# CliMA/ClimateParameterizations.jl

Measured on AMD Instinct MI355X. Metric: column-timesteps/sec (fwd+adjoint), 32-level wind-mixing NDE, higher is better.
Workload: dtype f32

## Files before the change

climateparameterizations.jl_amd/csrc/engine_regtile.hip:

```cpp
#include <cstdlib>
#include "engine_regtile.h"
#include "kernel_select.h"
#include "split_bf16.h"

typedef float f32x16 __attribute__((ext_vector_type(16)));

#ifdef COLNDE_STAMPS
__device__ unsigned long long g_rt_stamps[16];
#define RT_STAMP_DECL unsigned long long rs_t0 = 0, rs_acc[8] = {0, 0, 0, 0, 0, 0, 0, 0}; const unsigned long long rs_kk = __builtin_amdgcn_s_memtime(), rs_rr = __builtin_amdgcn_s_memrealtime()
#define RT_STAMP_BEGIN() do { __builtin_amdgcn_sched_barrier(0); rs_t0 = __builtin_amdgcn_s_memtime(); __builtin_amdgcn_sched_barrier(0); } while (0)
#define RT_STAMP(i) do { __builtin_amdgcn_sched_barrier(0); unsigned long long t_ = __builtin_amdgcn_s_memtime(); rs_acc[i] += t_ - rs_t0; rs_t0 = t_; __builtin_amdgcn_sched_barrier(0); } while (0)
#define RT_STAMP_FLUSH() do { if (blockIdx.x == 0 && threadIdx.x == 0) { for (int q_ = 0; q_ < 8; q_++) g_rt_stamps[q_] = rs_acc[q_]; g_rt_stamps[8] = __builtin_amdgcn_s_memtime() - rs_kk; g_rt_stamps[9] = __builtin_amdgcn_s_memrealtime() - rs_rr; } } while (0)
#else
#define RT_STAMP_DECL
#define RT_STAMP_BEGIN()
#define RT_STAMP(i)
#define RT_STAMP_FLUSH()
#endif
typedef float f32x4v __attribute__((ext_vector_type(4)));
typedef float f32x2v __attribute__((ext_vector_type(2)));

#define RHO0(r) (((r) & 3) + 8 * ((r) >> 2))
#ifndef RT16_WAVES
#define RT16_WAVES 8
// ... 803 lines not shown
                gg[r] = (r == 0 && h == 0) ? 0.0f : (d[r] - dd[r]) * 32.0f;
                sums[q] += d[r] * d[r];
                sums[3 + q] += gg[r] * gg[r];
            }
            if (add) {
                const f32x16 gu_ = shift_up(gg, h, 0.0f);
#pragma unroll
                for (int r = 0; r < 16; r++)
                    lam[RT_LAM(q * 16 + r, lane)] += 2.0f * lw.w[q] * d[r] + 2.0f * lw.w[3 + q] * 32.0f * (gg[r] - gu_[r]);
            }
        }
    };
    inject(0, false);

    auto load_z1 = [&](int step, int st, int n, f32x16 (&Z)[2], f32x16 (&Dz)[2]) {
        size_t rec = (size_t)step * 4 + st;
#ifdef RT_ABL_Z1_CACHED
        { int z_ = 0; asm volatile("" : "+v"(z_)); rec = (size_t)z_; }
#endif
        const float* srcz = tpz + rec * RT_TAPEZ;
        auto fill = [&](const float* src, f32x16 (&T)[2]) {
#pragma unroll
            for (int t = (13 * n) >> 2; t <= (13 * n + 12) >> 2; t++)
#pragma unroll
                for (int c = 0; c < 2; c++) {
                    const f32x4v v = RT_TAPE_LOAD4(src + (2 * t + c) * 256);
#pragma unroll
                    for (int e = 0; e < 4; e++) {
                        const int G = 2 * (4 * t + e - 13 * n) + c;
                        if ((4 * t + e) / 13 == n && G < 25) T[G >> 4][G & 15] = v[e];
                    }
                }
        };
        fill(srcz, Z);
        if (RT_ZRICH) fill(srcz + RT_TAPEZ_HALF, Dz);
    };

    auto load_z2 = [&](int step, int st, int n, f32x16& Z) {
        const float* srcz = tpz + ((size_t)step * 4 + st) * RT_TAPEZ + RT_Z2OFF + n * 3 * 256;
#pragma unroll
        for (int grp = 0; grp < 3; grp++) {
            const f32x4v v = RT_TAPE_LOAD4(srcz + grp * 256);
#pragma unroll
            for (int e = 0; e < 4; e++) Z[4 * grp + e] = (4 * grp + e < 10) ? v[e] : 0.0f;
        }
#pragma unroll
        for (int r = 12; r < 16; r++) Z[r] = 0.0f;
    };

    auto load_x = [&](int step, int st) {
        const float* src = tp + ((size_t)step * 4 + st) * 3072;
#pragma unroll
        for (int q = 0; q < 3; q++)
#pragma unroll
            for (int g = 0; g < 4; g++) {
                const f32x4v v = RT_TAPE_LOAD4(src + (q * 4 + g) * 256);
                X[q][4 * g] = v[0]; X[q][4 * g + 1] = v[1]; X[q][4 * g + 2] = v[2]; X[q][4 * g + 3] = v[3];
            }
    };

    for (int iv = n_save - 2; iv >= 0; iv--) {
        const float dt = (save_times[iv + 1] - save_times[iv]) / (float)substeps;
        inject(iv + 1, true);
        for (int s = substeps - 1; s >= 0; s--) {
            const int step = iv * substeps + s;
#pragma nounroll
            for (int st = 3; st >= 0; st--) {
                const float cwl = (st == 0 || st == 3) ? dt / 6.0f : dt / 3.0f;
                const float cwx = st == 3 ? 0.0f : (st == 2 ? dt : 0.5f * dt);
                RT_STAMP_BEGIN();
                f32x16 A1[2], D1[2];
                f32x16 A1n[2], D1n[2];
#pragma unroll
                for (int r = 9; r < 16; r++) { A1[1][r] = 0.0f; D1[1][r] = 0.0f; A1n[1][r] = 0.0f; D1n[1][r] = 0.0f; }
                load_x(step, st);
                f32x16 dOk[3];
                {
                    f32x16 kb[3];
#pragma unroll
                    for (int q = 0; q < 3; q++)
#pragma unroll
                        for (int r = 0; r < 16; r++) kb[q][r] = cwl * lam[RT_LAM(q * 16 + r, lane)] + cwx * xb[q][r];
                    rt_physics_vjp(m, X, kb, h, xb);
#pragma unroll
                    for (int q = 0; q < 3; q++) dOk[q] = kb[q];
                }
                RT_STAMP(0);
                float* dst = tp2 + ((size_t)step * 4 + st) * RT_TAPE2;
                float carry[2] = {0.0f, 0.0f};
#pragma unroll
                for (int n = 0; n < 3; n++) {
                    const f32x16 dOn = dOk[n];
                    if (ZT) {
                        if (n == 0) {
                            load_z1(step, st, 0, A1, D1);
#ifdef COLNDE_STAMPS
                            asm volatile("s_waitcnt vmcnt(0)" ::: "memory");
                            RT_STAMP(7);
#endif
                            if (!RT_ZRICH) {
#pragma unroll
                                for (int G = 0; G < 24; G += 4) rt_act_pair4_at<ACT>(A1, D1, G);
                                rt_act_pair_at<ACT>(A1, D1, 24);
                            }
                        }
                    } else {
#pragma unroll
                        for (int t = 0; t < 2; t++) {
                            f32x16 acc;
#pragma unroll
                            for (int r = 0; r < 16; r++) acc[r] = (t * 16 + r < 25) ? wl[RT_B1C + n * 50 + 2 * (t * 16 + r) + h] : 0.0f;
                            const int base = a1n[t] + n * 50 * RT_LD1;
                            acc = rt_chain<48, RT_ADJ_CH>(wl, acc, [=](int k) { return base + (k >> 4) * 32 + RHO0(k & 15); },
                                                          [&](int k) { return X[k >> 4][k & 15]; });
#pragma unroll
                            for (int r = 0; r < 16; r++) {
                                float av = 0.0f, dv = 0.0f;
                                if (t * 16 + r < 25) rt_act_pair<ACT>(acc[r], av, dv);
                                A1[t][r] = av;
                                D1[t][r] = dv;
                            }
                        }
                    }
                    RT_STAMP(1);
                    f32x16 Z2;
                    if (ZT && RT_Z2TAPE) load_z2(step, st, n, Z2);
                    else {
                        f32x16 acc;
#pragma unroll
                        for (int r = 0; r < 16; r++) acc[r] = r < 10 ? wl[RT_B2C + n * 20 + 2 * r + h] : 0.0f;
                        const int base2 = a2b + n * 20 * RT_LD2;
                        Z2 = rt_chain<25, 5>(wl, acc, [=](int k) { return base2 + 2 * k; },
                                             [&](int k) { return A1[k >> 4][k & 15]; });
                    }
                    RT_STAMP(2);
                    {
#ifndef RT_ABL_NO_OUTER
                        const f32x16 TA = rt_transpose(tb, dOn, wbase, rbase);
                        b3acc[n] += rt_sum16(TA);
#endif
                        f32x16 A2;
#pragma unroll
                        for (int r = 0; r < 16; r += 4) {
                            f32x2v a0 = {0.0f, 0.0f}, d0 = {0.0f, 0.0f}, a1 = {0.0f, 0.0f}, d1 = {0.0f, 0.0f};
                            if (r < 8) rt_act_pair4<ACT>((f32x2v){Z2[r], Z2[r + 1]}, (f32x2v){Z2[r + 2], Z2[r + 3]}, a0, d0, a1, d1);
                            else if (r == 8) rt_act_pair2<ACT>((f32x2v){Z2[8], Z2[9]}, a0, d0);
                            A2[r] = a0.x; A2[r + 1] = a0.y; A2[r + 2] = a1.x; A2[r + 3] = a1.y;
                            Z2[r] = d0.x; Z2[r + 1] = d0.y; Z2[r + 2] = d1.x; Z2[r + 3] = d1.y;
                        }
#ifndef RT_ABL_NO_OUTER
                        const f32x16 TB = rt_transpose(tb, A2, wbase, rbase);
#ifdef RT_OUTER_SPLIT
                        if constexpr (SPLIT) gW3[n] = rt_outer_split(gW3[n], rt_split_tile(TA), rt_split_tile(TB));
                        else
#endif
                        gW3[n] = rt_outer(gW3[n], TA, TB);
#else
                        gW3[n][0] += A2[0];
#endif
                    }
                    {
                        const int base = b3T + n * 31 * RT_LD3;
                        const f32x16 da = rt_chain<16, 8>(wl, (f32x16)(0.0f), [=](int k) { return base + RHO0(k) * RT_LD3; },
                                                          [&](int k) { return dOn[k]; });
#pragma unroll
                        for (int r = 0; r < 16; r++) Z2[r] = da[r] * Z2[r];
                    }
                    RT_STAMP(3);
                    if (ZT && n < 2) load_z1(step, st, n + 1, A1n, D1n);
#ifndef RT_LPIPE
#define RT_LPIPE 1
#endif
                    u32x4 Lr[9];
                    const u32x4* lg = nullptr;
                    if constexpr (SPLIT) {
                        int lz = lane;
                        asm volatile("" : "+v"(lz));
                        lg = reinterpret_cast<const u32x4*>(wimg + RT_ASIMG_OFF + RT_ASIMG_L) + n * 9 * 64 + lz;
#pragma unroll
                        for (int u = 0; u < (RT_LPIPE ? 3 : 9); u++) Lr[u] = lg[u * 64];
                    }
#ifdef RT_ABL_NO_OUTER
                    gW2[n][0][0] += Z2[0] * A1[0][0]; gW2[n][1][0] += Z2[1] * A1[1][0];
#else
                    {
                        const f32x16 TA = rt_transpose(tb, Z2, wbase, rbase);
                        b2acc[n] += rt_sum16(TA);
#ifdef RT_OUTER_SPLIT
                        Bf3x2 TAs;
                        if constexpr (SPLIT) TAs = rt_split_tile(TA);
#endif
#pragma unroll
                        for (int t = 0; t < 2; t++) {
                            const f32x16 TB = rt_transpose(tb, A1[t], wbase, rbase);
#ifdef RT_OUTER_SPLIT
                            if constexpr (SPLIT) gW2[n][t] = rt_outer_split(gW2[n][t], TAs, rt_split_tile(TB));
                            else
#endif
                            gW2[n][t] = rt_outer(gW2[n][t], TA, TB);
                        }
                    }
#endif
                    RT_STAMP(4);
#pragma unroll
                    for (int t = 0; t < 2; t++) {
                        const int base = b2T[t] + n * 20 * RT_LD2;
                        const f32x16 da = rt_chain<10, 10>(wl, (f32x16)(0.0f), [=](int k) { return base + 2 * k * RT_LD2; },
                                                           [&](int k) { return Z2[k]; });
#pragma unroll
                        for (int r = 0; r < 16; r++) D1[t][r] = da[r] * D1[t][r];
                    }
                    auto store_delta = [&] {
#pragma unroll
                    for (int g = 0; g < 25; g++) {
                        const int G = 25 * n + g;
                        if ((G & 3) == 0 && g + 3 < 25) {
                            const f32x4v v = {D1[g >> 4][g & 15], D1[(g + 1) >> 4][(g + 1) & 15], D1[(g + 2) >> 4][(g + 2) & 15],
                                              D1[(g + 3) >> 4][(g + 3) & 15]};
                            RT_NT_STORE4(dst + (G >> 2) * 256, v);
                        }
                    }
                    if (n == 0) carry[0] = D1[1][8];
                    if (n == 1) {
                        RT_NT_STORE4(dst + 6 * 256, ((f32x4v){carry[0], D1[0][0], D1[0][1], D1[0][2]}));
                        carry[0] = D1[1][7];
                        carry[1] = D1[1][8];
                    }
                    if (n == 2) {
                        RT_NT_STORE4(dst + 12 * 256, ((f32x4v){carry[0], carry[1], D1[0][0], D1[0][1]}));
                        RT_NT_STORE4(dst + 18 * 256, ((f32x4v){D1[1][6], D1[1][7], D1[1][8], 0.0f}));
                    }
                    };
#ifndef RT_ABL_NO_TAPE2
                    if constexpr (!SPLIT) store_delta();
#endif
                    RT_STAMP(5);
                    if constexpr (SPLIT) {
                        const u32x4* hm = reinterpret_cast<const u32x4*>(rt_smem) + lane;
#pragma unroll
                        for (int c = 0; c < 3; c++) {
                            if (RT_LPIPE && c < 2) {
#pragma unroll
                                for (int u = 0; u < 3; u++) Lr[3 * (c + 1) + u] = lg[(3 * (c + 1) + u) * 64];
                            }
                            float d8[8];
#pragma unroll
                            for (int u = 0; u < 8; u++) d8[u] = D1[(8 * c + u) >> 4][(8 * c + u) & 15];
                            const Bf3 Bc = bf3_split8(d8);
#pragma unroll
                            for (int q = 0; q < 3; q++) {
                                const int G = n * 9 + c * 3 + q, slot = c * 3 + q;
                                const u32x4 Ah = hm[(G * 2) * 64], Am = hm[(G * 2 + 1) * 64];
                                if (ZT && !RT_ZRICH && n < 2 && slot >= 2) {
                                    if (slot < 8) rt_act_pair4_at<ACT>(A1n, D1n, 4 * (slot - 2));
                                    else rt_act_pair_at<ACT>(A1n, D1n, 24);
                                }
                                xb[q] = mfma_bf(Am, Bc.m, xb[q]);
                                xb[q] = mfma_bf(Ah, Bc.l, xb[q]);
                                xb[q] = mfma_bf(Am, Bc.h, xb[q]);
                                xb[q] = mfma_bf(Ah, Bc.m, xb[q]);
                                xb[q] = mfma_bf(Ah, Bc.h, xb[q]);
                                xb[q] = mfma_bf(Lr[slot], Bc.h, xb[q]);
                                RT_SCHED_FENCE();
                            }
                        }
                        const float* left = rt_smem + RT_ASIMG_LEFT + (n * 2 + h) * 96 + i_;
#pragma unroll
                        for (int q = 0; q < 3; q++) xb[q] = mfma32(left[q * 32], D1[1][8], xb[q]);
                        store_delta();
                    } else
#pragma unroll
                    for (int q = 0; q < 3; q++) {
                        const int base = b1T + q * 32 + n * 50 * RT_LD1;
                        xb[q] = rt_chain_fill<25, 5>(wl, xb[q], [=](int g) { return base + 2 * g * RT_LD1; },
                                                     [&](int g) { return D1[g >> 4][g & 15]; },
                                                     [&](int c) {
                                                         if (ZT && !RT_ZRICH && n < 2 && (q > 0 || c > 0)) {
#pragma unroll
                                                             for (int G = 0; G < 24; G += 4)
                                                                 if ((G >> 2) * 2 + 2 == q * 5 + c)
                                                                     rt_act_pair4_at<ACT>(A1n, D1n, G);
                                                             if (q * 5 + c == 14) rt_act_pair_at<ACT>(A1n, D1n, 24);
                                                         }
                                                     });
                    }
                    if (ZT && n < 2) {
#pragma unroll
                        for (int t = 0; t < 2; t++) { A1[t] = A1n[t]; D1[t] = D1n[t]; }
                    }
                }
                RT_STAMP(6);
#pragma unroll
                for (int q = 0; q < 3; q++) xbs[q] += xb[q];
            }
#pragma unroll
            for (int q = 0; q < 3; q++) {
#pragma unroll
                for (int r = 0; r < 16; r++) lam[RT_LAM(q * 16 + r, lane)] += xbs[q][r];
                xbs[q] = (f32x16)(0.0f);
            }
        }
    }

#ifndef COLNDE_STAMPS_FWD
    RT_STAMP_FLUSH();
#endif
    float* out = slab + (size_t)tile * (m.n_params + 8);
    const int r_j = (j & 3) + 4 * (j >> 3), h_j = (j >> 2) & 1;
#pragma unroll
    for (int n = 0; n < 3; n++) {
        if (r_j < 10) {
            const int f2 = 2 * r_j + h_j;
#pragma unroll
            for (int r = 0; r < 16; r++) {
                const int face = RHO0(r) + 4 * h;
                if (face >= 1) out[n * m.net_size + m.w_off[2] + f2 * 31 + face - 1] = gW3[n][r];
            }
        }
#pragma unroll
        for (int t = 0; t < 2; t++) {
            const int Gp = t * 16 + r_j;
            if (Gp < 25) {
                const int f1 = 2 * Gp + h_j;
#pragma unroll
                for (int r = 0; r < 10; r++) out[n * m.net_size + m.w_off[1] + f1 * 20 + 2 * r + h] = gW2[n][t][r];
            }
        }
        const float s2 = b2acc[n] + swap32(b2acc[n], h), s3 = b3acc[n] + swap32(b3acc[n], h);
        if (h == 0) {
            if (r_i < 10) out[n * m.net_size + m.b_off[1] + 2 * r_i + h_i] = s2;
            if (i_ >= 1) out[n * m.net_size + m.b_off[2] + i_ - 1] = s3;
        }
    }
#pragma unroll
    for (int q = 0; q < 6; q++) {
        float v = sums[q];
        for (int off = 32; off > 0; off >>= 1) v += __shfl_down(v, off);
        if (lane == 0) out[m.n_params + q] = v;
    }
}

#define RT_DW1_LDS (4 * 2048)
__global__ void __launch_bounds__(256)
rt_dw1_kernel(DevModel m, const float* __restrict__ tape, const float* __restrict__ tape2, long n_items,
              float* __restrict__ slab_rows) {
    const int lane = threadIdx.x & 63, wave = __builtin_amdgcn_readfirstlane(threadIdx.x >> 6);
    const int j = lane & 31, h = lane >> 5;
    float* buf = rt_smem + wave * RT_DW1_LDS;
    const long gw = (long)blockIdx.x * RT_WAVES + wave, GW = (long)gridDim.x * RT_WAVES;
    f32x16 gW1[5][3];
#pragma unroll
    for (int mt = 0; mt < 5; mt++)
#pragma unroll
        for (int q = 0; q < 3; q++) gW1[mt][q] = (f32x16)(0.0f);
    float b1acc[5] = {0, 0, 0, 0, 0};
    const int NQ = gw < n_items ? 4 * (int)((n_items - gw + GW - 1) / GW) : 0;
    const int soff = ((lane >> 1) & 3) * 256 + ((lane & 1) * 32 + (lane >> 3)) * 4;
    auto issue = [&](int Q, int ring) {
        const int Qc = Q < NQ ? Q : NQ - 1;
        const size_t item = (size_t)(gw + (long)(Qc >> 2) * GW);
        const float* sx = tape + item * 3072 + soff + (Qc & 3) * 32;
        const float* sz = tape2 + item * RT_TAPE2 + soff + (Qc & 3) * 32;
#pragma unroll
        for (int T = 0; T < 3; T++) __builtin_amdgcn_global_load_lds(sx + T * 1024, buf + ring * 2048 + T * 256, 16, 0, RT_DMA_AUX);
#pragma unroll
        for (int T = 0; T < 5; T++) __builtin_amdgcn_global_load_lds(sz + T * 1024, buf + ring * 2048 + (3 + T) * 256, 16, 0, RT_DMA_AUX);
    };
    const float* rd = buf + h * 32 + j;
    float op[2][8][4];
    auto read_set = [&](int set, int ring) {
#pragma unroll
        for (int T = 0; T < 8; T++)
#pragma unroll
            for (int s = 0; s < 4; s++) op[set][T][s] = rd[ring * 2048 + T * 256 + 64 * s];
    };
    if (NQ > 0) {
        issue(0, 0);
        issue(1, 1);
        issue(2, 2);
        asm volatile("s_waitcnt vmcnt(16)" ::: "memory");
        read_set(0, 0);
    }
    for (int Qb = 0; Qb < NQ; Qb += 4) {
#pragma unroll
        for (int u = 0; u < 4; u++) {
            const int cur = u & 1;
#pragma unroll
            for (int s = 0; s < 4; s++)
#pragma unroll
                for (int q = 0; q < 3; q++) gW1[0][q] = mfma32(op[cur][3][s], op[cur][q][s], gW1[0][q]);
            b1acc[0] += (op[cur][3][0] + op[cur][3][1]) + (op[cur][3][2] + op[cur][3][3]);
            __builtin_amdgcn_sched_barrier(0);
            issue(Qb + u + 3, (u + 3) & 3);
            asm volatile("s_waitcnt vmcnt(16)" ::: "memory");
            read_set(cur ^ 1, (u + 1) & 3);
            __builtin_amdgcn_sched_barrier(0);
#pragma unroll
            for (int mt = 1; mt < 5; mt++) {
#pragma unroll
                for (int s = 0; s < 4; s++)
#pragma unroll
                    for (int q = 0; q < 3; q++) gW1[mt][q] = mfma32(op[cur][3 + mt][s], op[cur][q][s], gW1[mt][q]);
                b1acc[mt] += (op[cur][3 + mt][0] + op[cur][3 + mt][1]) + (op[cur][3 + mt][2] + op[cur][3 + mt][3]);
            }
            __builtin_amdgcn_sched_barrier(0);
        }
    }
    asm volatile("s_waitcnt vmcnt(0)" ::: "memory");
    float* out = slab_rows + (size_t)gw * (m.n_params + 8);
#pragma unroll
    for (int mt = 0; mt < 5; mt++) {
#pragma unroll
        for (int r = 0; r < 16; r++) {
            const int G = mt * 16 + r;
            if (G < 75) {
                const int n = G / 25, f = 2 * (G % 25) + h;
#pragma unroll
                for (int q = 0; q < 3; q++) out[n * m.net_size + m.w_off[0] + (q * 32 + j) * 50 + f] = gW1[mt][q][r];
            }
        }
        const float s1 = b1acc[mt] + swap32(b1acc[mt], h);
        const int r_j = (j & 3) + 4 * (j >> 3), h_j = (j >> 2) & 1;
        const int G = mt * 16 + r_j;
        if (h == 0 && G < 75) out[(G / 25) * m.net_size + m.b_off[0] + 2 * (G % 25) + h_j] = s1;
    }
}

__global__ void __launch_bounds__(256)
rt_dw1_split_kernel(DevModel m, const float* __restrict__ tape, const float* __restrict__ tape2, long n_items,
                    float* __restrict__ slab_rows) {
    const int lane = threadIdx.x & 63, wave = __builtin_amdgcn_readfirstlane(threadIdx.x >> 6);
    const int j = lane & 31, h = lane >> 5;
    float* buf = rt_smem + wave * RT_DW1_LDS;
    const long gw = (long)blockIdx.x * RT_WAVES + wave, GW = (long)gridDim.x * RT_WAVES;
    f32x16 gW1[5][3];
#pragma unroll
    for (int mt = 0; mt < 5; mt++)
#pragma unroll
        for (int q = 0; q < 3; q++) gW1[mt][q] = (f32x16)(0.0f);
    float b1acc[5] = {0, 0, 0, 0, 0};
    const int NQ = gw < n_items ? 4 * (int)((n_items - gw + GW - 1) / GW) : 0;
    const int soff = ((lane >> 1) & 3) * 256 + ((lane & 1) * 32 + (lane >> 3)) * 4;
    auto issue = [&](int Q, int ring) {
        const int Qc = Q < NQ ? Q : NQ - 1;
        const size_t item = (size_t)(gw + (long)(Qc >> 2) * GW);
        const float* sx = tape + item * 3072 + soff + (Qc & 3) * 32;
        const float* sz = tape2 + item * RT_TAPE2 + soff + (Qc & 3) * 32;
#pragma unroll
        for (int T = 0; T < 3; T++) __builtin_amdgcn_global_load_lds(sx + T * 1024, buf + ring * 2048 + T * 256, 16, 0, RT_DMA_AUX);
#pragma unroll
        for (int T = 0; T < 5; T++) __builtin_amdgcn_global_load_lds(sz + T * 1024, buf + ring * 2048 + (3 + T) * 256, 16, 0, RT_DMA_AUX);
    };
    const float* rd = buf + h * 2048 + j;
    float raw[2][8][8];
    auto read_half = [&](int set, int slot0) {
#pragma unroll
        for (int T = 0; T < 8; T++)
#pragma unroll
            for (int c = 0; c < 8; c++) raw[set][T][c] = rd[slot0 * 2048 + T * 256 + c * 32];
    };
    if (NQ > 0) {
        issue(0, 0);
        issue(1, 1);
        issue(2, 2);
        issue(3, 3);
        asm volatile("s_waitcnt vmcnt(16)" ::: "memory");
        read_half(0, 0);
        asm volatile("s_waitcnt lgkmcnt(0)" ::: "memory");
        issue(4, 0);
        issue(5, 1);
    }
    for (int Qb = 0; Qb < NQ; Qb += 4) {
#pragma unroll
        for (int u = 0; u < 2; u++) {
            const int cur = u;
            asm volatile("s_waitcnt vmcnt(16)" ::: "memory");
            read_half(cur ^ 1, 2 * (u ^ 1));
            __builtin_amdgcn_sched_barrier(0);
            Bf3 X[3];
#pragma unroll
            for (int q = 0; q < 3; q++) X[q] = bf3_split8(raw[cur][q]);
            __builtin_amdgcn_sched_barrier(0);
            asm volatile("s_waitcnt lgkmcnt(0)" ::: "memory");
            issue(Qb + 2 * u + 6, 2 * (u ^ 1));
            issue(Qb + 2 * u + 7, 2 * (u ^ 1) + 1);
            __builtin_amdgcn_sched_barrier(0);
#pragma unroll
            for (int mt = 0; mt < 5; mt++) {
                const Bf3 Z = bf3_split8(raw[cur][3 + mt]);
#pragma unroll
                for (int q = 0; q < 3; q++) gW1[mt][q] = mfma_bf3(Z, X[q], gW1[mt][q]);
                const float* z = raw[cur][3 + mt];
                b1acc[mt] += ((z[0] + z[1]) + (z[2] + z[3])) + ((z[4] + z[5]) + (z[6] + z[7]));
            }
            __builtin_amdgcn_sched_barrier(0);
        }
    }
    asm volatile("s_waitcnt vmcnt(0)" ::: "memory");
    float* out = slab_rows + (size_t)gw * (m.n_params + 8);
#pragma unroll
    for (int mt = 0; mt < 5; mt++) {
#pragma unroll
        for (int r = 0; r < 16; r++) {
            const int G = mt * 16 + r;
            if (G < 75) {
                const int n = G / 25, f = 2 * (G % 25) + h;
#pragma unroll
                for (int q = 0; q < 3; q++) out[n * m.net_size + m.w_off[0] + (q * 32 + j) * 50 + f] = gW1[mt][q][r];
            }
        }
        const float s1 = b1acc[mt] + swap32(b1acc[mt], h);
        const int r_j = (j & 3) + 4 * (j >> 3), h_j = (j >> 2) & 1;
        const int G = mt * 16 + r_j;
        if (h == 0 && G < 75) out[(G / 25) * m.net_size + m.b_off[0] + 2 * (G % 25) + h_j] = s1;
    }
}

typedef float f32x4t __attribute__((ext_vector_type(4)));

__device__ __forceinline__ f32x4t mfma16t(float a, float b, f32x4t c) {
    return __builtin_amdgcn_mfma_f32_16x16x4f32(a, b, c, 0, 0, 0);
}

__device__ __forceinline__ f32x4t mfma16_bf(u32x4 a, u32x4 b, f32x4t c) {
    return __builtin_amdgcn_mfma_f32_16x16x32_bf16(__builtin_bit_cast(bf16x8, a), __builtin_bit_cast(bf16x8, b), c, 0, 0, 0);
}
__device__ __forceinline__ f32x4t mfma16_bf3(const Bf3& a, const Bf3& b, f32x4t c) {
    c = mfma16_bf(a.m, b.m, c);
    c = mfma16_bf(a.l, b.h, c);
    c = mfma16_bf(a.h, b.l, c);
    c = mfma16_bf(a.m, b.h, c);
    c = mfma16_bf(a.h, b.m, c);
    c = mfma16_bf(a.h, b.h, c);
    return c;
}
__device__ __forceinline__ Bf3 rt16_ldA(const u32x4* simg, int G, int lane) {
    Bf3 a;
    a.h = simg[(G * 3 + 0) * 64 + lane];
    a.m = simg[(G * 3 + 1) * 64 + lane];
    a.l = simg[(G * 3 + 2) * 64 + lane];
    return a;
}

__device__ __forceinline__ float rot_dn16(float x, int lane) { return __shfl(x, (lane + 48) & 63); }
__device__ __forceinline__ float rot_up16(float x, int lane) { return __shfl(x, (lane + 16) & 63); }

struct V16 { f32x4t t[2]; };

__device__ __forceinline__ V16 shift_down16(const V16& T, int lane, float below) {
    const int g = lane >> 4;
    const float r0 = rot_dn16(T.t[0][3], lane), r1 = rot_dn16(T.t[1][3], lane);
    V16 o;
    o.t[0][0] = g == 0 ? below : r0;
    o.t[1][0] = g == 0 ? r0 : r1;
#pragma unroll
    for (int tau = 0; tau < 2; tau++) { o.t[tau][1] = T.t[tau][0]; o.t[tau][2] = T.t[tau][1]; o.t[tau][3] = T.t[tau][2]; }
    return o;
}

__device__ __forceinline__ V16 shift_up16(const V16& T, int lane, float above) {
    const int g = lane >> 4;
    const float r0 = rot_up16(T.t[0][0], lane), r1 = rot_up16(T.t[1][0], lane);
    V16 o;
    o.t[0][3] = g == 3 ? r1 : r0;
    o.t[1][3] = g == 3 ? above : r1;
#pragma unroll
    for (int tau = 0; tau < 2; tau++) { o.t[tau][0] = T.t[tau][1]; o.t[tau][1] = T.t[tau][2]; o.t[tau][2] = T.t[tau][3]; }
    return o;
}

template <int N, int CH, class AF, class BF>
__device__ __forceinline__ f32x4t rt16_chain(const float* wl, f32x4t acc, AF aidx, BF bval) {
    float a[2][CH];
#pragma unroll
    for (int u = 0; u < CH; u++)
        if (u < N) a[0][u] = wl[aidx(u)];
    RT_SCHED_FENCE();
    __builtin_amdgcn_s_setprio(1);
#pragma unroll
    for (int c = 0; c * CH < N; c++) {
#pragma unroll
        for (int u = 0; u < CH; u++)
            if ((c + 1) * CH + u < N) a[(c + 1) & 1][u] = wl[aidx((c + 1) * CH + u)];
#pragma unroll
        for (int u = 0; u < CH; u++)
            if (c * CH + u < N) acc = mfma16t(a[c & 1][u], bval(c * CH + u), acc);
        RT_SCHED_FENCE();
    }
    __builtin_amdgcn_s_setprio(0);
    return acc;
}

template <int N, int CH, int NV, class AF, class BF, class FF>
__device__ __forceinline__ f32x4t rt16_chain_fill(const float* wl, f32x4t acc, AF aidx, BF bval, FF fill) {
    float a[2][CH];
#pragma unroll
    for (int u = 0; u < CH; u++)
        if (u < N) a[0][u] = wl[aidx(u)];
    RT_SCHED_HARD();
    fill();
#pragma unroll
    for (int c = 0; c * CH < N; c++) {
#pragma unroll
        for (int u = 0; u < CH; u++)
            if ((c + 1) * CH + u < N) a[(c + 1) & 1][u] = wl[aidx((c + 1) * CH + u)];
#pragma unroll
        for (int u = 0; u < CH; u++)
            if (c * CH + u < N) acc = mfma16t(a[c & 1][u], bval(c * CH + u), acc);
    }
#pragma unroll
    for (int i = 0; i < N; i++) {
        __builtin_amdgcn_sched_group_barrier(0x008, 1, 0);
        __builtin_amdgcn_sched_group_barrier(0x100, 1, 0);
        __builtin_amdgcn_sched_group_barrier(0x402, NV, 0);
    }
    RT_SCHED_HARD();
    return acc;
}

template <int ACT, bool SPLIT = false>
__global__ void __launch_bounds__(512)
rt16_forward_kernel(DevModel m, const float* __restrict__ wimg, const float* __restrict__ x0, const float* __restrict__ bcs,
                    const float* __restrict__ save_times, int n_save, int substeps, float* __restrict__ sol,
                    float* __restrict__ tape, float* __restrict__ tapez, int n_col) {
    float* wl = rt_smem;
    const float* bl = wl;
    const u32x4* simg = reinterpret_cast<const u32x4*>(rt_smem);
    if constexpr (SPLIT) {
        const unsigned* src = reinterpret_cast<const unsigned*>(wimg + RT_SIMG_OFF);
        unsigned* dst = reinterpret_cast<unsigned*>(rt_smem);
        for (int e = threadIdx.x; e < RT_SIMG_WORDS / 4; e += blockDim.x)
            reinterpret_cast<u32x4*>(dst)[e] = reinterpret_cast<const u32x4*>(src)[e];
        for (int e = threadIdx.x; e < RT_IMG_FLOATS - RT_B1C; e += blockDim.x) wl[RT_SIMG_WORDS + e] = wimg[RT_B1C + e];
        bl = wl + RT_SIMG_WORDS - RT_B1C;
    } else {
        for (int e = threadIdx.x; e < RT_IMG_FLOATS; e += blockDim.x) wl[e] = wimg[e];
    }
    __syncthreads();
    const int lane = threadIdx.x & 63, wave = threadIdx.x >> 6;
    const int j = lane & 15, g = lane >> 4;
    const int wt = blockIdx.x * (blockDim.x >> 6) + wave;
    const int tile32 = wt >> 1, half = wt & 1;
    if (tile32 * 32 >= n_col) return;
    const int col = wt * 16 + j;
    const bool valid = col < n_col;
    const int colc = min(col, n_col - 1);
    const int i_ = lane & 15, g_i = i_ >> 2, r_i = i_ & 3;
    int a1b[10];
#pragma unroll
    for (int t = 0; t < 10; t++) {
        const int Q = 4 * t + r_i, f = 4 * (Q % 13) + g_i;
        const int row = (Q < 39 && f < 50) ? (Q / 13) * 50 + f : 0;
        a1b[t] = RT_W1C + row * RT_LD1 + 4 * g;
    }
    int a2b[2], a2l[2], a3b[2];
#pragma unroll
    for (int u = 0; u < 2; u++) {
        const int Q2 = 4 * u + r_i;
        const int row2 = Q2 < 5 ? 4 * Q2 + g_i : 0;
        a2b[u] = RT_W2C + row2 * RT_LD2 + g;
        a2l[u] = RT_W2C + row2 * RT_LD2 + (g < 2 ? 48 + g : 50);
        a3b[u] = RT_W3C + (16 * u + i_ - 1) * RT_LD3 + g;
    }
    RtBC bc;
    float bc5;
    {
        const float* bp = bcs + (size_t)colc * 6;
        bc.b[0] = bp[0]; bc.t[0] = bp[1]; bc.b[1] = bp[2]; bc.t[1] = bp[3]; bc.b[2] = bp[4]; bc5 = bp[5];
        bc.t[2] = bc5;
    }
    V16 Xn[3];
#pragma unroll
    for (int q = 0; q < 3; q++)
#pragma unroll
        for (int tau = 0; tau < 2; tau++) {
            const f32x4v v = *reinterpret_cast<const f32x4v*>(x0 + (size_t)colc * 96 + q * 32 + 16 * tau + 4 * g);
            Xn[q].t[tau] = v;
            if (sol && valid) *reinterpret_cast<f32x4v*>(sol + ((size_t)col * n_save) * 96 + q * 32 + 16 * tau + 4 * g) = v;
        }
    const int n_steps = (n_save - 1) * substeps;
    RT_STAMP_DECL;
#ifdef COLNDE_STAMPS_FWD
    const unsigned long long rs_k0 = __builtin_amdgcn_s_memtime(), rs_r0 = __builtin_amdgcn_s_memrealtime();
#endif
    float* tp = tape ? tape + (size_t)tile32 * n_steps * 4 * 3072 + ((g >> 1) * 64 + j + 16 * half + 32 * (g & 1)) * 4 : nullptr;
    float* tz = tapez ? tapez + (size_t)tile32 * n_steps * 4 * RT_TAPEZ + ((g >> 1) * 64 + j + 16 * half + 32 * (g & 1)) * 4 : nullptr;
    const float Nz = 32.0f;
    struct { float cU, sU, cV, sV, cB, sB, kE, oE, cE, nA, nB, f0, f1, f2; } pc;
    {
        const float L2E = 1.4426950408889634f;
        pc.cU = m.sig_u * Nz; pc.sU = m.sig_u * m.eps; pc.cV = m.sig_v * Nz; pc.sV = m.sig_v * m.eps; pc.cB = m.B * Nz; pc.sB = m.B * m.eps;
        pc.kE = 2.0f * m.inv_dRi * L2E; pc.oE = -2.0f * m.Ric * m.inv_dRi * L2E; pc.cE = 30.0f * L2E;
        pc.nA = -0.5f * m.nu_minus; pc.nB = m.nu0 + 0.5f * m.nu_minus;
        pc.f0 = -m.cs[0] * Nz; pc.f1 = -m.cs[1] * Nz; pc.f2 = -m.cs[2] * m.inv_Pr * Nz;
    }
    int step = 0;
    for (int iv = 0; iv < n_save - 1; iv++) {
        const float t0 = save_times[iv];
        const float dt = (save_times[iv + 1] - t0) / (float)substeps;
        for (int s = 0; s < substeps; s++, step++) {
            const float ts = t0 + (float)s * dt;
            V16 Xs[3], Kacc[3];
#pragma unroll
            for (int q = 0; q < 3; q++) { Xs[q] = Xn[q]; Kacc[q].t[0] = (f32x4t)(0.0f); Kacc[q].t[1] = (f32x4t)(0.0f); }
#pragma nounroll
            for (int st = 0; st < 4; st++) {
                const float ca = st == 0 ? 0.0f : (st == 3 ? 1.0f : 0.5f);
                const float cb = (st == 0 || st == 3) ? 1.0f / 6.0f : 1.0f / 3.0f;
                RT_STAMP_BEGIN();
                if (tp) {
                    float* o = tp + ((size_t)step * 4 + st) * 3072;
#pragma unroll
                    for (int q = 0; q < 3; q++)
#pragma unroll
                        for (int tau = 0; tau < 2; tau++) *reinterpret_cast<f32x4v*>(o + (q * 4 + 2 * tau) * 256) = Xs[q].t[tau];
                }
                bc.t[2] = rt_top_flux(m, bc5, ts + ca * dt);
                RT_STAMP(0);
                f32x4t A1[10];
                int lz = lane;
                if constexpr (SPLIT) asm volatile("" : "+v"(lz));
                if constexpr (SPLIT) {
#pragma unroll
                    for (int t = 0; t < 10; t++)
#pragma unroll
                        for (int r = 0; r < 4; r++) {
                            const int Q = 4 * t + r;
                            A1[t][r] = Q < 39 ? bl[RT_B1C + (Q / 13) * 50 + min(4 * (Q % 13) + g, 49)] : 0.0f;
                        }
                    Bf3 Apf = rt16_ldA(simg, 0, lz);
#pragma unroll
                    for (int q = 0; q < 3; q++) {
                        const float x8[8] = {Xs[q].t[0][0], Xs[q].t[0][1], Xs[q].t[0][2], Xs[q].t[0][3], Xs[q].t[1][0], Xs[q].t[1][1], Xs[q].t[1][2], Xs[q].t[1][3]};
                        const Bf3 XB = bf3_split8(x8);
#pragma unroll
                        for (int t = 0; t < 10; t++) {
                            const Bf3 Ac = Apf;
                            const int nx = q * 10 + t + 1;
                            if (nx < 30) Apf = rt16_ldA(simg, 3 * (nx % 10) + nx / 10, lz);
                            auto finish = [&](int tt) {
                                float* oz = tz ? tz + ((size_t)step * 4 + st) * RT_TAPEZ + 2 * tt * 256 : nullptr;
                                if (tz && !RT_ZRICH) *reinterpret_cast<f32x4v*>(oz) = A1[tt];
#pragma unroll
                                for (int r = 0; r < 4; r++) asm volatile("" : "+v"(A1[tt][r]));
                                if (RT_ZRICH && tz) {
                                    f32x2v a0, d0, a1, d1;
                                    rt_act_pair4<ACT>((f32x2v){A1[tt][0], A1[tt][1]}, (f32x2v){A1[tt][2], A1[tt][3]}, a0, d0, a1, d1);
                                    A1[tt] = (f32x4t){a0.x, a0.y, a1.x, a1.y};
                                    *reinterpret_cast<f32x4v*>(oz) = A1[tt];
                                    *reinterpret_cast<f32x4v*>(oz + RT_TAPEZ_HALF) = (f32x4v){d0.x, d0.y, d1.x, d1.y};
                                } else
                                A1[tt] = rt_act4<ACT>(A1[tt]);
#pragma unroll
                                for (int r = 0; r < 4; r++) asm volatile("" : "+v"(A1[tt][r]));
                            };
                            if (q == 2) RT_SCHED_HARD();
                            __builtin_amdgcn_s_setprio(1);
                            A1[t] = mfma16_bf3(Ac, XB, A1[t]);
                            __builtin_amdgcn_s_setprio(0);
                            if (q == 2) {
                                if (t > 0) {
                                    finish(t - 1);
#pragma unroll
                                    for (int u = 0; u < 6; u++) {
                                        __builtin_amdgcn_sched_group_barrier(0x008, 1, 0);
                                        __builtin_amdgcn_sched_group_barrier(0x402, 9, 0);
                                    }
                                }
                                RT_SCHED_HARD();
                                if (t == 9) finish(9);
                            } else
                                RT_SCHED_FENCE();
                        }
                    }
                } else {
                auto finish1 = [&](int tt) {
                    float* oz = tz ? tz + ((size_t)step * 4 + st) * RT_TAPEZ + 2 * tt * 256 : nullptr;
                    if (tz && !RT_ZRICH) *reinterpret_cast<f32x4v*>(oz) = A1[tt];
#pragma unroll
                    for (int r = 0; r < 4; r++) asm volatile("" : "+v"(A1[tt][r]));
                    if (RT_ZRICH && tz) {
                        f32x2v a0, d0, a1, d1;
                        rt_act_pair4<ACT>((f32x2v){A1[tt][0], A1[tt][1]}, (f32x2v){A1[tt][2], A1[tt][3]}, a0, d0, a1, d1);
                        A1[tt] = (f32x4t){a0.x, a0.y, a1.x, a1.y};
                        *reinterpret_cast<f32x4v*>(oz) = A1[tt];
                        *reinterpret_cast<f32x4v*>(oz + RT_TAPEZ_HALF) = (f32x4v){d0.x, d0.y, d1.x, d1.y};
                    } else
                    A1[tt] = rt_act4<ACT>(A1[tt]);
#pragma unroll
                    for (int r = 0; r < 4; r++) asm volatile("" : "+v"(A1[tt][r]));
                };
#pragma unroll
                for (int t = 0; t < 10; t++) {
                    f32x4t acc;
#pragma unroll
                    for (int r = 0; r < 4; r++) {
                        const int Q = 4 * t + r;
                        acc[r] = Q < 39 ? wl[RT_B1C + (Q / 13) * 50 + min(4 * (Q % 13) + g, 49)] : 0.0f;
                    }
                    const int base = a1b[t];
// ... 1932 lines not shown
```

Before: 191.7 million.

## Software-pipeline dW1 kernel: interleave bf16 splitting, LDS reads and refills with MFMAs

Restructures the rt_dw1_split_kernel main loop from per-quarter batch processing into a fine-grained software pipeline. Each of the five output row groups runs 18 MFMA slots, and into those slots it interleaves the LDS tile reads, the bf16 three-way splitting for the next iteration, the bias partial sums, and per-piece global-to-LDS refills. Loads are now issued in half-item units with a deeper ring and tuned vmcnt waits. The aim is to hide the VALU split work and memory latency behind matrix instructions, at the cost of much more complex scheduling and register pressure. It also adds optional timing stamps and probe modes, which are off by default.

```diff
diff --git a/climateparameterizations.jl_amd/csrc/engine_regtile.hip b/climateparameterizations.jl_amd/csrc/engine_regtile.hip
--- a/climateparameterizations.jl_amd/csrc/engine_regtile.hip
+++ b/climateparameterizations.jl_amd/csrc/engine_regtile.hip
@@ -1129,7 +1129,7 @@
         }
     }
 
-#ifndef COLNDE_STAMPS_FWD
+#if !defined(COLNDE_STAMPS_FWD) && !defined(COLNDE_STAMPS_DW1)
     RT_STAMP_FLUSH();
 #endif
     float* out = slab + (size_t)tile * (m.n_params + 8);
@@ -1253,9 +1253,28 @@
     }
 }
 
+#if defined(COLNDE_STAMPS) && defined(COLNDE_STAMPS_DW1)
+#define DW1_STAMP_DECL RT_STAMP_DECL
+#define DW1_STAMP_BEGIN() RT_STAMP_BEGIN()
+#define DW1_STAMP(i) RT_STAMP(i)
+#define DW1_STAMP_FLUSH() RT_STAMP_FLUSH()
+#else
+#define DW1_STAMP_DECL
+#define DW1_STAMP_BEGIN()
+#define DW1_STAMP(i)
+#define DW1_STAMP_FLUSH()
+#endif
+#ifndef RT_DW1_PROBE
+#define RT_DW1_PROBE 0
+#endif
+__device__ __forceinline__ void dw1_keep(const Bf3& b) {
+#pragma unroll
+    for (int p = 0; p < 4; p++) asm volatile("" ::"v"(b.h[p]), "v"(b.m[p]), "v"(b.l[p]));
+}
 __global__ void __launch_bounds__(256)
 rt_dw1_split_kernel(DevModel m, const float* __restrict__ tape, const float* __restrict__ tape2, long n_items,
                     float* __restrict__ slab_rows) {
+    DW1_STAMP_DECL;
     const int lane = threadIdx.x & 63, wave = __builtin_amdgcn_readfirstlane(threadIdx.x >> 6);
     const int j = lane & 31, h = lane >> 5;
     float* buf = rt_smem + wave * RT_DW1_LDS;
@@ -1266,63 +1285,142 @@
 #pragma unroll
         for (int q = 0; q < 3; q++) gW1[mt][q] = (f32x16)(0.0f);
     float b1acc[5] = {0, 0, 0, 0, 0};
-    const int NQ = gw < n_items ? 4 * (int)((n_items - gw + GW - 1) / GW) : 0;
-    const int soff = ((lane >> 1) & 3) * 256 + ((lane & 1) * 32 + (lane >> 3)) * 4;
-    auto issue = [&](int Q, int ring) {
-        const int Qc = Q < NQ ? Q : NQ - 1;
-        const size_t item = (size_t)(gw + (long)(Qc >> 2) * GW);
-        const float* sx = tape + item * 3072 + soff + (Qc & 3) * 32;
-        const float* sz = tape2 + item * RT_TAPE2 + soff + (Qc & 3) * 32;
-#pragma unroll
-        for (int T = 0; T < 3; T++) __builtin_amdgcn_global_load_lds(sx + T * 1024, buf + ring * 2048 + T * 256, 16, 0, RT_DMA_AUX);
-#pragma unroll
-        for (int T = 0; T < 5; T++) __builtin_amdgcn_global_load_lds(sz + T * 1024, buf + ring * 2048 + (3 + T) * 256, 16, 0, RT_DMA_AUX);
+    const int NH = gw < n_items ? 2 * (int)((n_items - gw + GW - 1) / GW) : 0;
+    const unsigned soff = ((lane >> 1) & 3) * 256 + ((lane & 1) * 32 + (lane >> 3)) * 4;
+    auto src_x = [&](int Hn) {
+        const int Hc = Hn < NH ? Hn : NH - 1;
+        return tape + ((size_t)(gw + (long)(Hc >> 1) * GW) * 3072 + (Hc & 1) * 64);
+    };
+    auto src_z = [&](int Hn) {
+        const int Hc = Hn < NH ? Hn : NH - 1;
+        return tape2 + ((size_t)(gw + (long)(Hc >> 1) * GW) * RT_TAPE2 + (Hc & 1) * 64);
+    };
+    auto fetch1 = [&](const float* s, int T, int RT, int par, int kk) {
+        __builtin_amdgcn_global_load_lds(s + (T * 1024 + kk * 32) + soff, buf + (2 * par + kk) * 2048 + RT * 256, 16, 0, RT_DMA_AUX);
+    };
+    auto fetch = [&](const float* s, int T, int RT, int par) {
+        fetch1(s, T, RT, par, 0);
+        fetch1(s, T, RT, par, 1);
+    };
+    auto refill1 = [&](int g, int u, int k, const float* sx3, const float* sz3, const float* sz2) {
+        if (g < 3 && k < 2) fetch1(sx3, g, g, u ^ 1, k);
+        else if (g < 4) fetch1(sz2, g + 1, 4 + g, u, k & 1);
+        else fetch1(sz3, 0, 3, u ^ 1, k & 1);
+    };
+    auto refill = [&](int g, int u, const float* sx3, const float* sz3, const float* sz2) {
+#pragma unroll
+        for (int k = 0; k < (g < 3 ? 4 : 2); k++) refill1(g, u, k, sx3, sz3, sz2);
     };
     const float* rd = buf + h * 2048 + j;
-    float raw[2][8][8];
-    auto read_half = [&](int set, int slot0) {
-#pragma unroll
-        for (int T = 0; T < 8; T++)
-#pragma unroll
-            for (int c = 0; c < 8; c++) raw[set][T][c] = rd[slot0 * 2048 + T * 256 + c * 32];
+    auto read_tile = [&](int par, int RT, float* raw) {
+#pragma unroll
+        for (int c = 0; c < 8; c++) raw[c] = rd[2 * par * 2048 + RT * 256 + c * 32];
     };
-    if (NQ > 0) {
-        issue(0, 0);
-        issue(1, 1);
-        issue(2, 2);
-        issue(3, 3);
+    Bf3 Xs[2][3], Zs[2];
+    float zs[2] = {0.0f, 0.0f};
+    float rawX[3][8];
+#if RT_DW1_PROBE == 1
+    Bf3 Pinv;
+#pragma unroll
+    for (int p = 0; p < 4; p++) { Pinv.h[p] = 0x3f803f80u + lane; Pinv.m[p] = 0x3b803b80u + lane; Pinv.l[p] = 0x37803780u + lane; }
+#endif
+    auto group = [&](auto PROD, int g, int u, const float* sx3, const float* sz3, const float* sz2) {
+        constexpr bool P = decltype(PROD)::value;
+        constexpr int first[6] = {0, 3, 6, 8, 10, 12};
+        const int nsteps = 10 + 2 * (first[g + 1] - first[g]), npieces = g < 3 ? 4 : 2;
+        const int zc = (g + u) & 1, zn = zc ^ 1;
+        float rawZ[8], ra = 0, rb = 0, la = 0, s4[4] = {0, 0, 0, 0};
+        auto half_pair = [&](const float* x, int p, int phase, Bf3& o) {
+            const float a = x[2 * p], b = x[2 * p + 1];
+            if (phase == 0) {
+                ra = a - __uint_as_float(__float_as_uint(a) & 0xffff0000u);
+                rb = b - __uint_as_float(__float_as_uint(b) & 0xffff0000u);
+                la = ra - __uint_as_float(__float_as_uint(ra) & 0xffff0000u);
+            } else {
+                const float lb = rb - __uint_as_float(__float_as_uint(rb) & 0xffff0000u);
+                o.h[p] = __builtin_amdgcn_perm(__float_as_uint(b), __float_as_uint(a), 0x07060302u);
+                o.m[p] = __builtin_amdgcn_perm(__float_as_uint(rb), __float_as_uint(ra), 0x07060302u);
+                o.l[p] = __builtin_amdgcn_perm(__float_as_uint(lb), __float_as_uint(la), 0x07060302u);
+            }
+        };
+        auto step = [&](int k) {
+#if RT_DW1_PROBE != 1
+            if (k < 8) half_pair(rawZ, k >> 1, k & 1, Zs[zn]);
+            else if (k == 8) {
+#pragma unroll
+                for (int c = 0; c < 4; c++) s4[c] = rawZ[2 * c] + rawZ[2 * c + 1];
+            } else if (k == 9) zs[zn] = (s4[0] + s4[1]) + (s4[2] + s4[3]);
+            else {
+                const int kp = first[g] + ((k - 10) >> 1);
+                half_pair(rawX[kp >> 2], kp & 3, k & 1, Xs[u ^ 1][kp >> 2]);
+            }
+#else
+            if (k == 0) Zs[zn] = Pinv;
+            if (k == 10 && g < 3) Xs[u ^ 1][g] = Pinv;
+#endif
+        };
+        DW1_STAMP_BEGIN();
+        if (P) {
+            if (g < 3) asm volatile("s_waitcnt vmcnt(28)" ::: "memory");
+            else asm volatile("s_waitcnt vmcnt(30)" ::: "memory");
+        }
+        DW1_STAMP(0);
+#pragma unroll
+        for (int i = 0; i < 18; i++) {
+            if (P) {
+#if RT_DW1_PROBE != 2
+                const Bf3 &A = Zs[zc], &B = Xs[u][i % 3];
+                f32x16& acc = gW1[g][i % 3];
+                switch (i / 3) {
+                case 0: acc = mfma_bf(A.m, B.m, acc); break;
+                case 1: acc = mfma_bf(A.l, B.h, acc); break;
+                case 2: acc = mfma_bf(A.h, B.l, acc); break;
+                case 3: acc = mfma_bf(A.m, B.h, acc); break;
+                case 4: acc = mfma_bf(A.h, B.m, acc); break;
+                default: acc = mfma_bf(A.h, B.h, acc); break;
+                }
+#else
+                if (i == 0) { dw1_keep(Zs[zc]); if (g == 0) { dw1_keep(Xs[u][0]); dw1_keep(Xs[u][1]); dw1_keep(Xs[u][2]); } }
+#endif
+                if (i == 0) b1acc[g] += zs[zc];
+            }
+#if RT_DW1_PROBE != 1
+            if (i == 0) {
+                if (g < 4) read_tile(u, 4 + g, rawZ);
+                else read_tile(u ^ 1, 3, rawZ);
+            }
+            if (i == 1 && g < 3) read_tile(u ^ 1, g, rawX[g]);
+#endif
+            if (i >= 18 - nsteps) step(i - (18 - nsteps));
+            if (i == 18 - npieces) asm volatile("s_waitcnt lgkmcnt(0)" ::: "memory");
+            if (i >= 18 - npieces) refill1(g, u, i - (18 - npieces), sx3, sz3, sz2);
+            if (P) __builtin_amdgcn_sched_barrier(0);
+        }
+        __builtin_amdgcn_sched_barrier(0);
+        DW1_STAMP(1);
+    };
+    if (NH > 0) {
+        const float *sx0 = src_x(0), *sz0 = src_z(0), *sx1 = src_x(1), *sz1 = src_z(1), *sx2 = src_x(2), *sz2 = src_z(2);
+#pragma unroll
+        for (int T = 0; T < 3; T++) fetch(sx0, T, T, 0);
+        fetch(sz0, 0, 3, 0);
+#pragma unroll
+        for (int g = 0; g < 5; g++) refill(g, 0, sx1, sz1, sz0);
         asm volatile("s_waitcnt vmcnt(16)" ::: "memory");
-        read_half(0, 0);
-        asm volatile("s_waitcnt lgkmcnt(0)" ::: "memory");
-        issue(4, 0);
-        issue(5, 1);
-    }
-    for (int Qb = 0; Qb < NQ; Qb += 4) {
+#pragma unroll
+        for (int g = 0; g < 5; g++) group(std::false_type{}, g, 1, sx2, sz2, sz1);
+    }
+    for (int H = 0; H < NH; H += 2) {
+        const float* sz2 = src_z(H + 2);
 #pragma unroll
         for (int u = 0; u < 2; u++) {
-            const int cur = u;
-            asm volatile("s_waitcnt vmcnt(16)" ::: "memory");
-            read_half(cur ^ 1, 2 * (u ^ 1));
-            __builtin_amdgcn_sched_barrier(0);
-            Bf3 X[3];
-#pragma unroll
-            for (int q = 0; q < 3; q++) X[q] = bf3_split8(raw[cur][q]);
-            __builtin_amdgcn_sched_barrier(0);
-            asm volatile("s_waitcnt lgkmcnt(0)" ::: "memory");
-            issue(Qb + 2 * u + 6, 2 * (u ^ 1));
-            issue(Qb + 2 * u + 7, 2 * (u ^ 1) + 1);
-            __builtin_amdgcn_sched_barrier(0);
-#pragma unroll
-            for (int mt = 0; mt < 5; mt++) {
-                const Bf3 Z = bf3_split8(raw[cur][3 + mt]);
-#pragma unroll
-                for (int q = 0; q < 3; q++) gW1[mt][q] = mfma_bf3(Z, X[q], gW1[mt][q]);
-                const float* z = raw[cur][3 + mt];
-                b1acc[mt] += ((z[0] + z[1]) + (z[2] + z[3])) + ((z[4] + z[5]) + (z[6] + z[7]));
-            }
-            __builtin_amdgcn_sched_barrier(0);
-        }
-    }
+            const float *sx3 = src_x(H + u + 3), *sz3 = src_z(H + u + 3);
+#pragma unroll
+            for (int g = 0; g < 5; g++) group(std::true_type{}, g, u, sx3, sz3, sz2);
+            sz2 = sz3;
+        }
+    }
+    DW1_STAMP_FLUSH();
     asm volatile("s_waitcnt vmcnt(0)" ::: "memory");
     float* out = slab_rows + (size_t)gw * (m.n_params + 8);
 #pragma unroll
```

Result: no change. 192.5 million, median of 6 (+0.4%).
